# SCUT-BIP-Lab/SplatCo

Hardware: AMD Instinct MI355X
Metric: rasterizer fwd+bwd Msplats/s @1080p; PSNR-match vs ref (higher is better)
Workload: dtype f32; 1 GPU; cfg1: 1M synthetic Gaussians (seed 0), 1 view 1920x1080 per GPU, GaussianRasterizer forward+backward, colors_precomp + scale/rotation path; gaussians=1000000, image=1920x1080, visible=1000000, parallelism=1 view per GPU (mv sharding)

## Files before the change

### splatco_amd/csrc/blend.hip

```cpp
#include <type_traits>

#include "common.h"

namespace scr {

typedef float v2f __attribute__((ext_vector_type(2)));

#ifdef SCR_BLEND_COUNT
__device__ __forceinline__ void count_sub_blocks(unsigned long long m, unsigned long long (&len)[4]) {
    len[0] += (m & 0x000000000f0f0f0full) != 0ull;
    len[1] += (m & 0x00000000f0f0f0f0ull) != 0ull;
    len[2] += (m & 0x0f0f0f0f00000000ull) != 0ull;
    len[3] += (m & 0xf0f0f0f000000000ull) != 0ull;
}
#define SCR_COUNT_SUB(m) (count_sub_blocks((m), sub_), count_sub_blocks((m), subc_))
#define SCR_COUNT_CHUNK_END(i)                                                                             \
    do {                                                                                                   \
        const unsigned long long a_ = subc_[0] > subc_[1] ? subc_[0] : subc_[1], b_ = subc_[2] > subc_[3] ? subc_[2] : subc_[3]; \
        cnt_[(i)] += a_ > b_ ? a_ : b_;                                                                    \
        subc_[0] = subc_[1] = subc_[2] = subc_[3] = 0;                                                     \
    } while (0)
#define SCR_COUNT_SUB_FLUSH(i_sum, i_max)                                                                  \
    do {                                                                                                   \
        cnt_[(i_sum)] += sub_[0] + sub_[1] + sub_[2] + sub_[3];                                            \
        const unsigned long long a_ = sub_[0] > sub_[1] ? sub_[0] : sub_[1], b_ = sub_[2] > sub_[3] ? sub_[2] : sub_[3]; \
        cnt_[(i_max)] += a_ > b_ ? a_ : b_;                                                                \
    } while (0)
#endif
#ifdef SCR_BLEND_COUNT
__device__ unsigned long long g_blend_counters[16];
#define SCR_COUNT(i, v) (cnt_[(i)] += (unsigned long long)(v))
#define SCR_COUNT_DECL unsigned long long cnt_[16] = {}, sub_[4] = {}, subc_[4] = {}
#define SCR_COUNT_FLUSH(lane)                                                        \
    if ((lane) == 0)                                                                 \
        for (int q_ = 0; q_ < 16; ++q_)                                              \
            if (cnt_[q_]) atomicAdd(&g_blend_counters[q_], cnt_[q_])
#else
#define SCR_COUNT(i, v) ((void)0)
#define SCR_COUNT_SUB(m) ((void)0)
#define SCR_COUNT_CHUNK_END(i) ((void)0)
#define SCR_COUNT_SUB_FLUSH(a, b) ((void)0)
#define SCR_COUNT_DECL ((void)0)
#define SCR_COUNT_FLUSH(lane) ((void)0)
#endif

__device__ __forceinline__ float fast_exp(float x) {
    const float p = x * 1.4426950408889634f;
    const float g = __builtin_amdgcn_exp2f(p);
    const float r = __builtin_fmaf(-p, 0.6931471805599453f, x);
    return __builtin_fmaf(g, r, g);
}

__device__ __forceinline__ uint32_t lanes_below(unsigned long long ballot) {
    return __builtin_amdgcn_mbcnt_hi((uint32_t)(ballot >> 32), __builtin_amdgcn_mbcnt_lo((uint32_t)ballot, 0u));
}

__global__ void __launch_bounds__(1024)
tile_order_kernel(int tiles, int gx, const uint32_t* __restrict__ ranges, uint32_t* __restrict__ order,
                  unsigned long long* __restrict__ ordered, unsigned long long* __restrict__ first) {
    __shared__ uint32_t hist[1024], start[1024], wsum[16];
    __shared__ uint32_t s_max, cnt[NUM_XCD];
    const int me = blockIdx.x;
    hist[threadIdx.x] = 0;
    if (threadIdx.x == 0) s_max = 1;
    if (threadIdx.x < NUM_XCD) cnt[threadIdx.x] = 0;
    __syncthreads();
    uint32_t mx = 0, mine[NUM_XCD] = {};
    for (int t = threadIdx.x; t < tiles; t += 1024) {
        const int x = xcd_of_tile(t, gx);
#pragma unroll
        for (int q = 0; q < NUM_XCD; ++q) mine[q] += x == q;
        if (x == me) mx = max(mx, ranges[2 * t + 1] - ranges[2 * t]);
    }
#pragma unroll
    for (int q = 0; q < NUM_XCD; ++q)
        if (mine[q]) atomicAdd(&cnt[q], mine[q]);
    if (mx) atomicMax(&s_max, mx);
    __syncthreads();
    uint32_t off = 0;
    for (int q = 0; q < me; ++q) off += cnt[q];
    const float scale = 1023.0f / (float)s_max;
    for (int t = threadIdx.x; t < tiles; t += 1024) {
        if (xcd_of_tile(t, gx) != me) continue;
        const uint32_t n = ranges[2 * t + 1] - ranges[2 * t];
        atomicAdd(&hist[1023 - min(1023u, (uint32_t)((float)n * scale))], 1u);
    }
    __syncthreads();
    {
        const int lane = threadIdx.x & 63, w = threadIdx.x >> 6;
        uint32_t v = hist[threadIdx.x], inc = v;
#pragma unroll
        for (int d = 1; d < 64; d <<= 1) {
            const uint32_t o = __shfl_up(inc, d, 64);
            if (lane >= d) inc += o;
        }
        if (lane == 63) wsum[w] = inc;
        __syncthreads();
        uint32_t base = 0;
        for (int q = 0; q < w; ++q) base += wsum[q];
        start[threadIdx.x] = base + inc - v;
    }
    __syncthreads();
    for (int t = threadIdx.x; t < tiles; t += 1024) {
        if (xcd_of_tile(t, gx) != me) continue;
        const uint32_t n = ranges[2 * t + 1] - ranges[2 * t];
        order[off + atomicAdd(&start[1023 - min(1023u, (uint32_t)((float)n * scale))], 1u)] = (uint32_t)t;
    }
    if (threadIdx.x == 0) {
        first[me] = off;
        if (me == NUM_XCD - 1) first[NUM_XCD] = off + cnt[me];
        if (me == 0) *ordered = 1;
    }
}

__device__ __forceinline__ int blend_tile(int slot, int tiles, const uint32_t* __restrict__ order,
                                          const unsigned long long* __restrict__ total) {
    const int xcd = slot % NUM_XCD, j = slot / NUM_XCD;
    if (total[2]) {
        const uint32_t f = (uint32_t)total[4 + xcd], e = (uint32_t)total[5 + xcd];
        return f + j < e ? (int)order[f + j] : -1;
    }
    const int chunk = (tiles + NUM_XCD - 1) / NUM_XCD;
    const int t = xcd * chunk + j;
    return j < chunk && t < tiles ? t : -1;
}

template <bool AUX>
__device__ __forceinline__ void masked_blend(unsigned long long live, float w, float cr, float cg, float cb, float z, float Tn,
                                             uint32_t j, float& C0, float& C1, float& C2, float& D, float& T, uint32_t& last) {
    if constexpr (AUX)
        asm volatile("s_mov_b64 exec, %6\n\t"
                     "v_fmac_f32_e32 %0, %7, %11\n\t"
                     "v_fmac_f32_e32 %1, %8, %11\n\t"
                     "v_fmac_f32_e32 %2, %9, %11\n\t"
                     "v_fmac_f32_e32 %3, %10, %11\n\t"
                     "v_mov_b32_e32 %4, %12\n\t"
                     "v_mov_b32_e32 %5, %13\n\t"
                     "s_mov_b64 exec, -1"
                     : "+v"(C0), "+v"(C1), "+v"(C2), "+v"(D), "+v"(T), "+v"(last)
                     : "s"(live), "v"(cr), "v"(cg), "v"(cb), "v"(z), "v"(w), "v"(Tn), "v"(j));
    else
        asm volatile("s_mov_b64 exec, %5\n\t"
                     "v_fmac_f32_e32 %0, %6, %9\n\t"
                     "v_fmac_f32_e32 %1, %7, %9\n\t"
                     "v_fmac_f32_e32 %2, %8, %9\n\t"
                     "v_mov_b32_e32 %3, %10\n\t"
                     "v_mov_b32_e32 %4, %11\n\t"
                     "s_mov_b64 exec, -1"
                     : "+v"(C0), "+v"(C1), "+v"(C2), "+v"(T), "+v"(last)
                     : "s"(live), "v"(cr), "v"(cg), "v"(cb), "v"(w), "v"(Tn), "v"(j));
}

constexpr int FCHUNK = 64;

template <bool SAFE, bool AUX>
__global__ void __launch_bounds__(64)
blend_forward_kernel(int W, int H, int gx, int tiles, const uint32_t* __restrict__ order, const unsigned long long* __restrict__ total,
                     const uint32_t* __restrict__ ranges,
                     const uint32_t* __restrict__ point_list, const uint8_t* __restrict__ qmask,
                     const float4* __restrict__ rec, const float* __restrict__ bg,
                     float* __restrict__ out_color, float* __restrict__ final_T,
                     uint32_t* __restrict__ n_contrib, float* __restrict__ out_depth, float* __restrict__ out_alpha) {
    constexpr int NF = AUX ? 6 : 5;
    __shared__ float4 sp[NF][FCHUNK / 2];
    const int quad = (blockIdx.x / NUM_XCD) & 3;
    const int t = blend_tile((int)(blockIdx.x % NUM_XCD + (blockIdx.x / (4 * NUM_XCD)) * NUM_XCD), tiles, order, total);
    if (t < 0) return;
    const int lane = threadIdx.x;
    const int px = (t % gx) * TILE + (quad & 1) * 8 + (lane & 7);
    const int py = (t / gx) * TILE + (quad >> 1) * 8 + (lane >> 3);
    const bool inside = px < W && py < H;
    const float pxf = (float)px, pyf = (float)py;
    const uint32_t lo = ranges[2 * t], n = ranges[2 * t + 1] - lo;
    unsigned long long done = lanes(!inside);
    SCR_COUNT_DECL;
    float T = 1.0f, C0 = 0.0f, C1 = 0.0f, C2 = 0.0f;
    float D = 0.0f;
    float c099 = 0.99f;
    asm volatile("" : "+v"(c099));
    uint32_t last = 0;

    uint32_t m_next = 0, id_next = 0;
    bool sel_cur = false;
    float4 r0 = make_float4(0, 0, 0, 0), r1 = r0;
    float r2x = 0.0f, r2y = 0.0f;
    auto load_mask_id = [&](uint32_t base, uint32_t& m, uint32_t& id) {
        uint32_t i = base + lane;
        bool have = i < n;
        m = have ? ((qmask[lo + i] >> quad) & 1u) : 0u;
        id = have ? point_list[lo + i] : 0u;
    };
    auto gather = [&](uint32_t m, uint32_t id) {
        sel_cur = m != 0;
        if (sel_cur) {
            r0 = rec[3 * (size_t)id];
            r1 = rec[3 * (size_t)id + 1];
            r2x = rec[3 * (size_t)id + 2].x;
            if (AUX) r2y = rec[3 * (size_t)id + 2].y;
        }
    };
    for (int i = lane; i < NF * (FCHUNK / 2); i += WAVE) (&sp[0][0])[i] = make_float4(0, 0, 0, 0);
    uint32_t m0, id0;
    load_mask_id(0, m0, id0);
    gather(m0, id0);
    load_mask_id(FCHUNK, m_next, id_next);

    for (uint32_t base = 0; base < n; base += FCHUNK) {
        const unsigned long long bal = __builtin_amdgcn_ballot_w64(sel_cur);
        const int cnt = __builtin_popcountll(bal);
        if (sel_cur) {
            const uint32_t pos = lanes_below(bal), q = pos >> 1, h = pos & 1;
            float* f0 = (float*)&sp[0][q];
            float* f1 = (float*)&sp[1][q];
            float* f2 = (float*)&sp[2][q];
            float* f3 = (float*)&sp[3][q];
            float* f4 = (float*)&sp[4][q];
            f0[h] = r0.x; f0[2 + h] = r0.y;
            f1[h] = r0.z; f1[2 + h] = r0.w;
            f2[h] = r1.x; f2[2 + h] = r1.y;
            f3[h] = r1.z; f3[2 + h] = r1.w;
            f4[h] = r2x;  f4[2 + h] = __uint_as_float(base + lane + 1);
            if (AUX) ((float*)&sp[NF - 1][q])[h] = r2y;
        }
        gather(m_next, id_next);
        load_mask_id(base + 2 * FCHUNK, m_next, id_next);
        __syncthreads();
        auto group = [&](const int k, auto npairs) {
            constexpr int NP = decltype(npairs)::value, NS = 2 * NP;
            v2f power[NP], al[NP];
            float4 p3[NP], p4[NP];
            float2 p5[NP];
#pragma unroll
            for (int h = 0; h < NP; ++h) {
                const int q = (k >> 1) + h;
                const float4 p0 = sp[0][q], p1 = sp[1][q], p2 = sp[2][q];
                p3[h] = sp[3][q];
                p4[h] = sp[4][q];
                if (AUX) p5[h] = *(const float2*)&sp[NF - 1][q];
                const v2f dx = v2f{p0.x, p0.y} - pxf, dy = v2f{p0.z, p0.w} - pyf;
                const v2f A = {p1.x, p1.y}, B = {p1.z, p1.w}, Cq = {p2.x, p2.y}, o = {p2.z, p2.w};
                power[h] = __builtin_elementwise_fma(dx, __builtin_elementwise_fma(A, dx, B * dy), (Cq * dy) * dy);
                al[h] = o * v2f{fast_exp(power[h].x), fast_exp(power[h].y)};
            }
            float alpha[NS], pw[NS], om[NS];
#pragma unroll
            for (int h = 0; h < NP; ++h) {
                alpha[2 * h] = vmin(c099, al[h].x); alpha[2 * h + 1] = vmin(c099, al[h].y);
                pw[2 * h] = power[h].x; pw[2 * h + 1] = power[h].y;
            }
#pragma unroll
            for (int u = 0; u < NS; ++u) om[u] = 1.0f - alpha[u];
            unsigned long long hit[NS], anyh = 0ull;
#pragma unroll
            for (int u = 0; u < NS; ++u) {
                hit[u] = (k + u < cnt) ? (lanes(!(pw[u] > 0.0f)) & lanes(!(alpha[u] < 1.0f / 255.0f))) : 0ull;
                anyh |= hit[u];
            }
#ifdef SCR_BLEND_COUNT
            for (int u = 0; u < NS; ++u)
                if (k + u < cnt) {
                    SCR_COUNT(0, 1);
                    SCR_COUNT(2, __builtin_popcountll(done & lanes(inside)));
                    SCR_COUNT(3, (anyh & ~done) == 0ull);
                }
#endif
            if ((anyh & ~done) == 0ull) return;
#pragma unroll
            for (int u = 0; u < NS; ++u) {
                const int h = u >> 1;
                const float cr = (u & 1) ? p3[h].y : p3[h].x, cg = (u & 1) ? p3[h].w : p3[h].z;
                const float cb = (u & 1) ? p4[h].y : p4[h].x, cj = (u & 1) ? p4[h].w : p4[h].z;
                const unsigned long long hm = hit[u] & ~done;
                const float Tn = T * om[u];
                const unsigned long long stop = lanes(Tn < 0.0001f) & hm;
                done |= stop;
                const unsigned long long live = hm & ~stop;
                SCR_COUNT(1, __builtin_popcountll(live));
                SCR_COUNT_SUB(live);
                const float w = alpha[u] * T;
                masked_blend<AUX>(live, w, cr, cg, cb, AUX ? ((u & 1) ? p5[h].y : p5[h].x) : 0.0f, Tn, __float_as_uint(cj),
                                  C0, C1, C2, D, T, last);
            }
        };
        int k = 0;
        for (; k + 2 < cnt; k += 4) group(k, std::integral_constant<int, 2>{});
        if (k < cnt) group(k, std::integral_constant<int, 1>{});
        SCR_COUNT_CHUNK_END(6);
        if (~done == 0ull) break;
        __syncthreads();
    }
    SCR_COUNT_SUB_FLUSH(4, 5);
    SCR_COUNT_FLUSH(lane);
    if (inside) {
        size_t pix = (size_t)py * W + px, hw = (size_t)H * W;
        out_color[pix] = __builtin_fmaf(T, bg[0], C0);
        out_color[hw + pix] = __builtin_fmaf(T, bg[1], C1);
        out_color[2 * hw + pix] = __builtin_fmaf(T, bg[2], C2);
        final_T[pix] = T;
        n_contrib[pix] = last;
        if (AUX) {
            out_depth[pix] = D;
            out_alpha[pix] = 1.0f - T;
        }
    }
}

#define SCR_DPP(d, s, ctrl) "v_add_f32_dpp " d ", " s ", " s " " ctrl "\n\t"
__device__ __forceinline__ void column_fold(float& s0, float& s1, float& s2, float t0, float t1, float t2) {
    asm volatile("s_nop 1\n\t"
                 SCR_DPP("%0", "%0", "row_shl:4 row_mask:0xf bank_mask:0x5")
                 SCR_DPP("%1", "%1", "row_shl:4 row_mask:0xf bank_mask:0x5")
                 SCR_DPP("%2", "%2", "row_shl:4 row_mask:0xf bank_mask:0x5")
                 SCR_DPP("%0", "%3", "row_shr:4 row_mask:0xf bank_mask:0xa")
                 SCR_DPP("%1", "%4", "row_shr:4 row_mask:0xf bank_mask:0xa")
                 SCR_DPP("%2", "%5", "row_shr:4 row_mask:0xf bank_mask:0xa")
                 SCR_DPP("%0", "%0", "quad_perm:[2,3,0,1] row_mask:0xf bank_mask:0xf")
                 SCR_DPP("%1", "%1", "quad_perm:[2,3,0,1] row_mask:0xf bank_mask:0xf")
                 SCR_DPP("%2", "%2", "quad_perm:[2,3,0,1] row_mask:0xf bank_mask:0xf")
                 SCR_DPP("%0", "%0", "quad_perm:[1,0,3,2] row_mask:0xf bank_mask:0xf")
                 SCR_DPP("%1", "%1", "quad_perm:[1,0,3,2] row_mask:0xf bank_mask:0xf")
                 SCR_DPP("%2", "%2", "quad_perm:[1,0,3,2] row_mask:0xf bank_mask:0xf")
                 "s_nop 1"
                 : "+v"(s0), "+v"(s1), "+v"(s2)
                 : "v"(t0), "v"(t1), "v"(t2));
}
constexpr int TCS = WAVE + 4;

struct PixState {
    float T, dLp0, dLp1, dLp2;
    float behind, last_alpha, d_last;
    float dLd, dLa;
};
template <bool SAFE, bool AUX>
__device__ __forceinline__ void splat_pixel_grad(PixState& s, float T, float4 b, float cb, float z, float G, float alpha,
                                                 unsigned long long hit, float& Y, float& w) {
#pragma clang fp contract(fast)
    w = alpha * T;
    s.behind = SAFE ? s.last_alpha * s.d_last + (1.0f - s.last_alpha) * s.behind : s.last_alpha * (s.d_last - s.behind) + s.behind;
    float d = b.z * s.dLp0 + b.w * s.dLp1 + cb * s.dLp2;
    if (AUX) d += z * s.dLd + s.dLa;
    if (SAFE) d = sel(hit, d, 0.0f);
    Y = G * (T * (d - s.behind));
    if (SAFE) Y = sel(hit, Y, 0.0f);
    s.last_alpha = alpha;
    s.d_last = d;
}
__device__ __forceinline__ void group_transmittance(float& T, const float (&om)[4], float (&Tu)[4]) {
#pragma clang fp contract(off)
    const float P = ((om[0] * om[1]) * om[2]) * om[3];
    float r = __builtin_amdgcn_rcpf(P);
    r = __builtin_fmaf(__builtin_fmaf(-P, r, 1.0f), r, r);
    const float q = T * r;
    Tu[3] = __builtin_fmaf(__builtin_fmaf(-q, P, T), r, q);
    Tu[2] = Tu[3] * om[3];
    Tu[1] = Tu[2] * om[2];
    Tu[0] = Tu[1] * om[1];
    T = Tu[3];
}

typedef float f4_t __attribute__((ext_vector_type(4)));
__device__ __forceinline__ void store16_dword_aligned(void* p, float4 v) {
    const f4_t q = {v.x, v.y, v.z, v.w};
    asm volatile("global_store_dwordx4 %0, %1, off" : : "v"(p), "v"(q) : "memory");
}

template <bool AUX> struct RecTail { float x; };
template <> struct RecTail<true> { float x, z; };
constexpr int BCH = 64;
constexpr int BWD_MIN_WAVES = 4;
constexpr int ACC_BUFS = 2;

constexpr int BWD_MIN_WAVES_AUX = 3;
template <bool SAFE, bool AUX>
__global__ void __launch_bounds__(256, AUX ? BWD_MIN_WAVES_AUX : BWD_MIN_WAVES)
blend_backward_kernel(int W, int H, int gx, int tiles, const uint32_t* __restrict__ order, const unsigned long long* __restrict__ total,
                      const uint32_t* __restrict__ ranges,
                      const uint32_t* __restrict__ point_list, const uint32_t* __restrict__ gm_index,
                      const uint2* __restrict__ gm_base,
                      const uint8_t* __restrict__ qmask, const float4* __restrict__ rec,
                      const float* __restrict__ bg, const float* __restrict__ final_T,
                      const uint32_t* __restrict__ n_contrib, const float* __restrict__ dL_dpix,
                      GradRec* __restrict__ grad_rec, unsigned long long* __restrict__ cut_key, unsigned long long stamp,
                      uint8_t* __restrict__ has_rec, const float* __restrict__ dL_ddepth, const float* __restrict__ dL_dalpha,
                      float* __restrict__ grad_z) {
    __shared__ float4 st[4][3][BCH + 4];
    __shared__ float4 accA[ACC_BUFS][4][BCH], accB[ACC_BUFS][4][BCH];
    __shared__ float accC[ACC_BUFS][4][BCH];
    __shared__ float accD[ACC_BUFS][4][BCH];
    __shared__ __attribute__((aligned(16))) float tr[4][8 * TCS];
    __shared__ uint32_t wave_max[4];
    const int t = blend_tile((int)blockIdx.x, tiles, order, total);
    if (t < 0) return;
    const uint32_t lo = ranges[2 * t], n = ranges[2 * t + 1] - lo;
    if (n == 0) return;
    const int wave = threadIdx.x >> 6, lane = threadIdx.x & 63;
    const int qx0 = (t % gx) * TILE + (wave & 1) * 8, qy0 = (t / gx) * TILE + (wave >> 1) * 8;
    const int px = qx0 + (lane >> 3), py = qy0 + (lane & 7);
    const bool inside = px < W && py < H;
    const float pxf = (float)px, pyf = (float)py;
    const float qx0f = (float)qx0, qy0f = (float)qy0;
    const size_t pix = (size_t)py * W + px, hw = (size_t)H * W;
    const uint32_t last = inside ? n_contrib[pix] : 0u;
    PixState ps;
    ps.T = inside ? final_T[pix] : 0.0f;
    ps.dLp0 = ps.dLp1 = ps.dLp2 = 0.0f;
    if (inside) {
        ps.dLp0 = dL_dpix[pix];
        ps.dLp1 = dL_dpix[hw + pix];
        ps.dLp2 = dL_dpix[2 * hw + pix];
    }
    ps.behind = (bg[0] * ps.dLp0 + bg[1] * ps.dLp1) + bg[2] * ps.dLp2;
    ps.last_alpha = ps.d_last = 0.0f;
    if (AUX) {
        ps.dLd = inside && dL_ddepth ? dL_ddepth[pix] : 0.0f;
        ps.dLa = inside && dL_dalpha ? dL_dalpha[pix] : 0.0f;
    }
    float c099 = 0.99f;
    asm volatile("" : "+v"(c099));
    SCR_COUNT_DECL;
    const int rcol = lane >> 3, rx = lane & 7;
    constexpr int WZ = AUX ? 3 : 0;
    float wgt[AUX ? 4 : 3][8];
#pragma unroll
    for (int y = 0; y < 8; ++y) {
        wgt[0][y] = 1.0f; wgt[1][y] = (float)y; wgt[2][y] = (float)(y * y);
        if (AUX) wgt[WZ][y] = 0.0f;
        if (rcol >= 4) {
            const bool in = qx0 + rx < W && qy0 + y < H;
            const size_t q = (size_t)(qy0 + y) * W + (size_t)(qx0 + rx);
#pragma unroll
            for (int c = 0; c < 3; ++c) wgt[c][y] = in ? dL_dpix[c * hw + q] : 0.0f;
            if (AUX) wgt[WZ][y] = in && dL_ddepth ? dL_ddepth[q] : 0.0f;
        }
    }
    const float xw = rcol < 4 ? (float)rx : 0.0f;
    float* const trw = &tr[wave][0];
    const float* const trr = trw + rcol * TCS + 8 * rx;
    const int rkind = rcol >= 4 ? 2 : (lane >> 2) & 1;
    const bool rstore = (lane & 3) == 0 && (rcol < 4 || ((lane >> 2) & 1) == 0);
    const bool rstore_z = AUX && (lane & 3) == 0 && rcol >= 4 && ((lane >> 2) & 1) == 1;
    const int rcu = rcol & 3;
    const unsigned long long rcu1 = lanes(rcu == 1), rcu2 = lanes(rcu == 2), rcu3 = lanes(rcu == 3);
    char* const accA0 = (char*)&accA[0][wave][0];
    char* const accB0 = (char*)&accB[0][wave][0];
    char* const rdst0 = rkind == 0 ? accA0 : rkind == 1 ? accA0 + 4 : accB0 + 8;
    char* const rdst1 = rkind == 0 ? accA0 + 8 : rkind == 1 ? accA0 + 12 : accB0 + 12;
    char* const rdst2 = rkind == 0 ? accB0 + 4 : rkind == 1 ? accB0 : (char*)&accC[0][wave][0];
    const uint32_t rstride2 = rkind == 2 ? 4u : 16u;
    constexpr uint32_t PAR_A = sizeof(float4) * 4 * BCH, PAR_C = sizeof(float) * 4 * BCH;
    const uint32_t rpar2 = rkind == 2 ? PAR_C : PAR_A;
    uint32_t wm = last;
#pragma unroll
    for (int d = 32; d > 0; d >>= 1) wm = max(wm, (uint32_t)__shfl_xor((int)wm, d, WAVE));
    if (lane == 0) wave_max[wave] = wm;
    if (lane < 9) st[wave][lane / 3][lane % 3] = make_float4(0, 0, 0, 0);
    __syncthreads();
    const uint32_t wmax0 = wave_max[0], wmax1 = wave_max[1], wmax2 = wave_max[2], wmax3 = wave_max[3];
    const uint32_t max_last = max(max(wmax0, wmax1), max(wmax2, wmax3));
    const uint32_t wave_last = wave == 0 ? wmax0 : wave == 1 ? wmax1 : wave == 2 ? wmax2 : wmax3;
    const int nround = (int)((n + BCH - 1) / BCH);
    const int live_top = max_last ? (int)((max_last - 1) / BCH) : -1;

    constexpr int CUT_MIN_ROUNDS = 3;
    const bool cut = nround - 1 - live_top >= CUT_MIN_ROUNDS;
    if (threadIdx.x == 0) {
        unsigned long long ck = ~0ull;
        if (cut) {
            const uint32_t idc = point_list[lo + (uint32_t)(live_top + 1) * BCH];
            ck = ((unsigned long long)__float_as_uint(rec[3 * (size_t)idc + 2].y) << 32) | idc;
            cut_key[tiles] = stamp;
        }
        cut_key[t] = ck;
    }
    const uint32_t tile_x = (uint32_t)(t % gx), tile_y = (uint32_t)(t / gx);
    auto gm_of = [&](uint32_t pos, uint32_t id) -> uint32_t {
        if (gm_index) return gm_index[pos];
        const uint2 b = gm_base[id];
        return b.x + tile_y * b.y + tile_x;
    };
    if (!cut && (AUX || wave < 3))
        for (int ci = nround - 1; ci > live_top; --ci) {
            const uint32_t i = (uint32_t)ci * BCH + lane;
            if (i < n && qmask[lo + i] != 0) {
                const uint32_t gmi = gm_of(lo + i, point_list[lo + i]);
                GradRec& gr = grad_rec[gmi];
                if (wave == 0) store16_dword_aligned(&gr.a, make_float4(0, 0, 0, 0));
                else if (wave == 1) store16_dword_aligned(&gr.b, make_float4(0, 0, 0, 0));
                else if (!AUX || wave == 2) gr.c = 0.0f;
                else grad_z[gmi] = 0.0f;
            }
        }

    uint32_t m_next = 0, id_next = 0, slot_next = 0;
    uint32_t m_cur = 0, slot_cur = 0, id_cur = 0;
    bool sel_cur = false;
    float4 r0 = make_float4(0, 0, 0, 0), r1 = r0;
    RecTail<AUX> r2 = {};
    auto load_meta = [&](int ci, uint32_t& m, uint32_t& id, uint32_t& slot) {
        const uint32_t i = (uint32_t)ci * BCH + lane;
        const bool have = ci >= 0 && i < n;
        m = have ? qmask[lo + i] : 0u;
        id = have ? point_list[lo + i] : 0u;
        slot = have ? gm_of(lo + i, id) : 0u;
    };
    auto gather = [&](int ci, uint32_t m, uint32_t id, uint32_t slot) {
        const uint32_t i = (uint32_t)ci * BCH + lane;
        sel_cur = ((m >> wave) & 1u) && i < wave_last;
        m_cur = m;
        slot_cur = slot;
        id_cur = id;
        if (sel_cur) {
            r0 = rec[3 * (size_t)id];
            r1 = rec[3 * (size_t)id + 1];
            r2.x = rec[3 * (size_t)id + 2].x;
            if constexpr (AUX) r2.z = rec[3 * (size_t)id + 2].y;
        }
    };
    if (live_top >= 0) {
        uint32_t m0, id0, sl0;
        load_meta(live_top, m0, id0, sl0);
        gather(live_top, m0, id0, sl0);
        load_meta(live_top - 1, m_next, id_next, slot_next);
    }
    for (int ci = live_top; ci >= 0; --ci) {
        const uint32_t base = (uint32_t)ci * BCH;
        const int last_rel = (int)last - (int)base;
        const unsigned long long bal = __builtin_amdgcn_ballot_w64(sel_cur);
        const int cnt = __builtin_popcountll(bal);
        if (sel_cur) {
            const uint32_t pos = lanes_below(bal);
            st[wave][0][pos + 3] = r0;
            st[wave][1][pos + 3] = r1;
            float r2z = 0.0f;
            if constexpr (AUX) r2z = r2.z;
            st[wave][2][pos + 3] = make_float4(r2.x, __uint_as_float((uint32_t)lane), r2z, 0.0f);
        }
        const uint32_t m_this = m_cur, slot_this = slot_cur, id_this = id_cur;
        gather(ci - 1, m_next, id_next, slot_next);
        load_meta(ci - 2, m_next, id_next, slot_next);
        const int par = ci & 1;
        auto group = [&](const int k, auto tail) {
            constexpr bool TAIL = decltype(tail)::value;
            float Y[4], Wt[4];
            uint32_t jj[4] = {0u, 0u, 0u, 0u};
            unsigned long long hits[4] = {0ull, 0ull, 0ull, 0ull};
            float4 ra[4], rb[4];
            float2 rc[4];
            float rz[4] = {0.0f, 0.0f, 0.0f, 0.0f};
#pragma unroll
            for (int u = 0; u < 4; ++u) {
                ra[u] = st[wave][0][k + 3 - u];
                rb[u] = st[wave][1][k + 3 - u];
                rc[u] = *(const float2*)&st[wave][2][k + 3 - u];
                if (AUX) rz[u] = st[wave][2][k + 3 - u].z;
            }
            float Gs[4], al[4], om[4], Tu[4];
#pragma unroll
            for (int u = 0; u < 4; ++u) {
                if (TAIL && k - u < 0) {
                    Gs[u] = al[u] = 0.0f;
                    om[u] = 1.0f;
                    SCR_COUNT(13, 1);
                    continue;
                }
                const float4 a = ra[u], b = rb[u];
                const uint32_t j = __float_as_uint(rc[u].y);
                const float dx = a.x - pxf, dy = a.y - pyf;
                const float power = __builtin_fmaf(dx, __builtin_fmaf(a.z, dx, a.w * dy), (b.x * dy) * dy);
                const float ar = b.y * fast_exp(power);
                const unsigned long long hit = lanes((int)j < last_rel) & lanes(!(power > 0.0f)) & lanes(!(ar < 1.0f / 255.0f));
                SCR_COUNT(8, 1);
                SCR_COUNT(9, __builtin_popcountll(hit));
                SCR_COUNT_SUB(hit);
                SCR_COUNT(10, __builtin_popcountll(lanes(!((int)j < last_rel)) & lanes(inside)));
                SCR_COUNT(11, __builtin_popcountll(lanes(!(power > 0.0f)) & lanes(!(ar < 1.0f / 255.0f)) & lanes(inside)));
                Gs[u] = sel(hit, ar, 0.0f);
                al[u] = vmin(c099, Gs[u]);
                om[u] = 1.0f - al[u];
                if (SAFE) hits[u] = hit;
                jj[u] = j;
            }
            group_transmittance(ps.T, om, Tu);
#pragma unroll
            for (int u = 0; u < 4; ++u) {
                if (TAIL && k - u < 0) {
                    Y[u] = Wt[u] = 0.0f;
                    continue;
                }
                splat_pixel_grad<SAFE, AUX>(ps, Tu[u], rb[u], rc[u].x, rz[u], Gs[u], al[u], hits[u], Y[u], Wt[u]);
            }
            float s0, s1, s2;
            {
                asm volatile("" ::: "memory");
#pragma unroll
                for (int u = 0; u < 4; ++u) {
                    trw[u * TCS + lane] = Y[u];
                    trw[(4 + u) * TCS + lane] = Wt[u];
                }
                asm volatile("" ::: "memory");
                const float4 va = *(const float4*)trr, vb = *(const float4*)(trr + 4);
                asm volatile("" ::: "memory");
                const float v[8] = {va.x, va.y, va.z, va.w, vb.x, vb.y, vb.z, vb.w};
                float e0 = wgt[0][0] * v[0], e1 = wgt[1][0] * v[0], e2 = wgt[2][0] * v[0];
                float o0 = wgt[0][1] * v[1], o1 = wgt[1][1] * v[1], o2 = wgt[2][1] * v[1];
#pragma unroll
                for (int y = 2; y < 8; y += 2) {
                    e0 = __builtin_fmaf(wgt[0][y], v[y], e0);
                    e1 = __builtin_fmaf(wgt[1][y], v[y], e1);
                    e2 = __builtin_fmaf(wgt[2][y], v[y], e2);
                    o0 = __builtin_fmaf(wgt[0][y + 1], v[y + 1], o0);
                    o1 = __builtin_fmaf(wgt[1][y + 1], v[y + 1], o1);
                    o2 = __builtin_fmaf(wgt[2][y + 1], v[y + 1], o2);
                }
                s0 = e0 + o0; s1 = e1 + o1; s2 = e2 + o2;
                float t0 = xw * s0;
                if (AUX) {
                    float e3 = wgt[WZ][0] * v[0], o3 = wgt[WZ][1] * v[1];
#pragma unroll
                    for (int y = 2; y < 8; y += 2) {
                        e3 = __builtin_fmaf(wgt[WZ][y], v[y], e3);
                        o3 = __builtin_fmaf(wgt[WZ][y + 1], v[y + 1], o3);
                    }
                    t0 = __builtin_fmaf(xw, s0, e3 + o3);
                }
                const float t1 = xw * t0, t2 = xw * s1;
                column_fold(s0, s1, s2, t0, t1, t2);
            }
            if (rstore && (!TAIL || k - rcu >= 0)) {
                const uint32_t jw = sel(rcu3, jj[3], sel(rcu2, jj[2], sel(rcu1, jj[1], jj[0])));
                *(float*)(rdst0 + par * PAR_A + jw * 16u) = s0;
                *(float*)(rdst1 + par * PAR_A + jw * 16u) = s1;
                *(float*)(rdst2 + par * rpar2 + jw * rstride2) = s2;
            }
            if (AUX && rstore_z && (!TAIL || k - rcu >= 0)) {
                const uint32_t jw = sel(rcu3, jj[3], sel(rcu2, jj[2], sel(rcu1, jj[1], jj[0])));
                accD[par][wave][jw] = s0;
            }
        };
        int k = cnt - 1;
        for (; k >= 3; k -= 4) group(k, std::false_type{});
        if (k >= 0) group(k, std::true_type{});
        SCR_COUNT_CHUNK_END(7);
        asm volatile("s_waitcnt lgkmcnt(0)" ::: "memory");
        if (lane < cnt) {
            const float4 ra = st[wave][0][lane + 3];
            const uint32_t j = __float_as_uint(st[wave][2][lane + 3].y);
            const float a = ra.x - qx0f, b = ra.y - qy0f;
            const float4 A = accA[par][wave][j], B = accB[par][wave][j];
            const float M0 = A.x, Mx = A.y, My = A.z, Mxx = A.w, Mxy = B.x, Myy = B.y;
            const float t1 = a * M0 - Mx, t2 = b * M0 - My;
            accA[par][wave][j] = make_float4(t1, t2, a * (t1 - Mx) + Mxx, (a * t2 - b * Mx) + Mxy);
            accB[par][wave][j] = make_float4(b * (t2 - My) + Myy, M0, B.z, B.w);
        }
        __syncthreads();
        if (wave < 3 && base + lane < n && m_this != 0) {
            const uint32_t i = base + lane;
            float4 r = make_float4(0, 0, 0, 0);
            auto part = [&](int w) {
                return wave == 0 ? accA[par][w][lane] : wave == 1 ? accB[par][w][lane]
                                                                  : make_float4(accC[par][w][lane], 0.0f, 0.0f, 0.0f);
            };
            if (((m_this >> 0) & 1u) && i < wmax0) { const float4 x = part(0); r.x += x.x; r.y += x.y; r.z += x.z; r.w += x.w; }
            if (((m_this >> 1) & 1u) && i < wmax1) { const float4 x = part(1); r.x += x.x; r.y += x.y; r.z += x.z; r.w += x.w; }
            if (((m_this >> 2) & 1u) && i < wmax2) { const float4 x = part(2); r.x += x.x; r.y += x.y; r.z += x.z; r.w += x.w; }
            if (((m_this >> 3) & 1u) && i < wmax3) { const float4 x = part(3); r.x += x.x; r.y += x.y; r.z += x.z; r.w += x.w; }
            GradRec& gr = grad_rec[slot_this];
            if (wave == 0) store16_dword_aligned(&gr.a, r);
            else if (wave == 1) store16_dword_aligned(&gr.b, r);
            else {
                gr.c = r.x;
                if (has_rec) has_rec[id_this] = 1;
            }
        }
        if (AUX && wave == 3 && base + lane < n && m_this != 0) {
            const uint32_t i = base + lane;
            float r = 0.0f;
            if (((m_this >> 0) & 1u) && i < wmax0) r += accD[par][0][lane];
            if (((m_this >> 1) & 1u) && i < wmax1) r += accD[par][1][lane];
            if (((m_this >> 2) & 1u) && i < wmax2) r += accD[par][2][lane];
            if (((m_this >> 3) & 1u) && i < wmax3) r += accD[par][3][lane];
            grad_z[slot_this] = r;
        }
    }
    SCR_COUNT_SUB_FLUSH(14, 15);
    SCR_COUNT_FLUSH(lane);
}

static int blend_slots_per_xcd(const Grid& g) {
    int cnt[NUM_XCD] = {};
    for (int t = 0; t < g.tiles; ++t) ++cnt[xcd_of_tile(t, g.gx)];
    int m = (g.tiles + NUM_XCD - 1) / NUM_XCD;
    for (int q = 0; q < NUM_XCD; ++q) m = cnt[q] > m ? cnt[q] : m;
    return m;
}

void launch_blend_forward(const KSettings& ks, const GeomView& gv, const BinView& bv, const ImgView& iv,
                          float* out_color, float* out_depth, float* out_alpha, bool longest_first, bool safe,
                          hipStream_t st) {
    Grid g(ks.H, ks.W);
    if (longest_first)
        tile_order_kernel<<<NUM_XCD, 1024, 0, st>>>(g.tiles, g.gx, gv.ranges, gv.tile_count, gv.total + 2, gv.total + 4);
    const bool aux = out_depth != nullptr;
    auto kernel = aux ? (safe ? blend_forward_kernel<true, true> : blend_forward_kernel<false, true>)
                      : (safe ? blend_forward_kernel<true, false> : blend_forward_kernel<false, false>);
    kernel<<<(unsigned)blend_slots_per_xcd(g) * NUM_XCD * 4, 64, 0, st>>>(
        ks.W, ks.H, g.gx, g.tiles, gv.tile_count, gv.total, gv.ranges, bv.point_list, bv.qmask, gv.rec, ks.bg, out_color, iv.final_T,
        iv.n_contrib, out_depth, out_alpha);
}

void launch_blend_backward(const KSettings& ks, const GeomView& gv, const BinView& bv, const ImgView& iv,
                           const float* dL_dcolor, const float* dL_ddepth, const float* dL_dalpha, GradRec* grad_rec,
                           float* grad_z, unsigned long long stamp, bool deep, bool flags, bool safe, hipStream_t st) {
    Grid g(ks.H, ks.W);
    const bool gm_from_base = deep;
    if (flags) { ZeroList z; z.add(gv.has_rec, ((size_t)gv.P + 3) / 4 * 4, st); launch_zero(z, st); }
    const bool aux = grad_z != nullptr;
    auto kernel = aux ? (safe ? blend_backward_kernel<true, true> : blend_backward_kernel<false, true>)
                      : (safe ? blend_backward_kernel<true, false> : blend_backward_kernel<false, false>);
    kernel<<<(unsigned)blend_slots_per_xcd(g) * NUM_XCD, 256, 0, st>>>(
        ks.W, ks.H, g.gx, g.tiles, gv.tile_count, gv.total, gv.ranges, bv.point_list, gm_from_base ? nullptr : bv.gm_index, gv.gm_base,
        bv.qmask, gv.rec, ks.bg,
        iv.final_T, iv.n_contrib, dL_dcolor, grad_rec, iv.cut_key, stamp, flags ? gv.has_rec : nullptr, dL_ddepth, dL_dalpha,
        grad_z);
}

}

#ifdef SCR_BLEND_COUNT
extern "C" int scr_tool_blend_counters(unsigned long long* out16, int reset) {
    if (out16 && hipMemcpyFromSymbol(out16, HIP_SYMBOL(scr::g_blend_counters), 16 * 8) != hipSuccess) return 1;
    if (reset) {
        unsigned long long z[16] = {};
        if (hipMemcpyToSymbol(HIP_SYMBOL(scr::g_blend_counters), z, 16 * 8) != hipSuccess) return 1;
    }
    return 0;
}
#endif
```

Before: 1095 Msplats/s.

## Read per-lane Gaussian slot from LDS, batch masked combine, split transpose layout

Adds three compile-time options to the backward blend kernel, all enabled by default (SCR_BWD_ITEMS=14). Each lane reads its slot index directly from the staged LDS record instead of a chain of selects. The four per-wave partial accumulators are combined with a single exec-masked inline-asm add sequence instead of branchy conditional adds. The transpose scratch buffer uses a split column layout to change LDS bank mapping. It also extends the debug counter set. The inline asm with exec manipulation risks correctness and register pressure, and the new layout could change bank conflicts either way.

```diff
diff --git a/splatco_amd/csrc/blend.hip b/splatco_amd/csrc/blend.hip
--- a/splatco_amd/csrc/blend.hip
+++ b/splatco_amd/csrc/blend.hip
@@ -28,12 +28,13 @@
     } while (0)
 #endif
 #ifdef SCR_BLEND_COUNT
-__device__ unsigned long long g_blend_counters[16];
+constexpr int SCR_NCOUNT = 20;
+__device__ unsigned long long g_blend_counters[SCR_NCOUNT];
 #define SCR_COUNT(i, v) (cnt_[(i)] += (unsigned long long)(v))
-#define SCR_COUNT_DECL unsigned long long cnt_[16] = {}, sub_[4] = {}, subc_[4] = {}
+#define SCR_COUNT_DECL unsigned long long cnt_[SCR_NCOUNT] = {}, sub_[4] = {}, subc_[4] = {}
 #define SCR_COUNT_FLUSH(lane)                                                        \
     if ((lane) == 0)                                                                 \
-        for (int q_ = 0; q_ < 16; ++q_)                                              \
+        for (int q_ = 0; q_ < SCR_NCOUNT; ++q_)                                              \
             if (cnt_[q_]) atomicAdd(&g_blend_counters[q_], cnt_[q_])
 #else
 #define SCR_COUNT(i, v) ((void)0)
@@ -324,7 +325,15 @@
                  : "+v"(s0), "+v"(s1), "+v"(s2)
                  : "v"(t0), "v"(t1), "v"(t2));
 }
+#ifndef SCR_BWD_ITEMS
+#define SCR_BWD_ITEMS 14
+#endif
+constexpr bool BWD_LANE_POS = (SCR_BWD_ITEMS & 2) != 0, BWD_BATCH_COMBINE = (SCR_BWD_ITEMS & 4) != 0,
+               BWD_TR_SPLIT = (SCR_BWD_ITEMS & 8) != 0;
+
 constexpr int TCS = WAVE + 4;
+constexpr int TR_WORDS = BWD_TR_SPLIT ? 8 * WAVE + 4 : 8 * TCS;
+__device__ __forceinline__ constexpr int tr_col(int c) { return BWD_TR_SPLIT ? WAVE * (c >> 1) + (c & 1) * (4 * WAVE + 4) : c * TCS; }
 
 struct PixState {
     float T, dLp0, dLp1, dLp2;
@@ -364,6 +373,51 @@
     asm volatile("global_store_dwordx4 %0, %1, off" : : "v"(p), "v"(q) : "memory");
 }
 
+__device__ __forceinline__ void masked_add4(float4& r, const float4 (&x)[4], const unsigned long long (&c)[4]) {
+    unsigned long long keep;
+    asm volatile("s_mov_b64 %4, exec\n\t"
+                 "s_mov_b64 exec, %5\n\t"
+                 "v_add_f32_e32 %0, %0, %9\n\t"
+                 "v_add_f32_e32 %1, %1, %10\n\t"
+                 "v_add_f32_e32 %2, %2, %11\n\t"
+                 "v_add_f32_e32 %3, %3, %12\n\t"
+                 "s_mov_b64 exec, %6\n\t"
+                 "v_add_f32_e32 %0, %0, %13\n\t"
+                 "v_add_f32_e32 %1, %1, %14\n\t"
+                 "v_add_f32_e32 %2, %2, %15\n\t"
+                 "v_add_f32_e32 %3, %3, %16\n\t"
+                 "s_mov_b64 exec, %7\n\t"
+                 "v_add_f32_e32 %0, %0, %17\n\t"
+                 "v_add_f32_e32 %1, %1, %18\n\t"
+                 "v_add_f32_e32 %2, %2, %19\n\t"
+                 "v_add_f32_e32 %3, %3, %20\n\t"
+                 "s_mov_b64 exec, %8\n\t"
+                 "v_add_f32_e32 %0, %0, %21\n\t"
+                 "v_add_f32_e32 %1, %1, %22\n\t"
+                 "v_add_f32_e32 %2, %2, %23\n\t"
+                 "v_add_f32_e32 %3, %3, %24\n\t"
+                 "s_mov_b64 exec, %4"
+                 : "+v"(r.x), "+v"(r.y), "+v"(r.z), "+v"(r.w), "=&s"(keep)
+                 : "s"(c[0]), "s"(c[1]), "s"(c[2]), "s"(c[3]),
+                   "v"(x[0].x), "v"(x[0].y), "v"(x[0].z), "v"(x[0].w), "v"(x[1].x), "v"(x[1].y), "v"(x[1].z), "v"(x[1].w),
+                   "v"(x[2].x), "v"(x[2].y), "v"(x[2].z), "v"(x[2].w), "v"(x[3].x), "v"(x[3].y), "v"(x[3].z), "v"(x[3].w));
+}
+__device__ __forceinline__ void masked_add4(float& r, const float (&x)[4], const unsigned long long (&c)[4]) {
+    unsigned long long keep;
+    asm volatile("s_mov_b64 %1, exec\n\t"
+                 "s_mov_b64 exec, %2\n\t"
+                 "v_add_f32_e32 %0, %0, %6\n\t"
+                 "s_mov_b64 exec, %3\n\t"
+                 "v_add_f32_e32 %0, %0, %7\n\t"
+                 "s_mov_b64 exec, %4\n\t"
+                 "v_add_f32_e32 %0, %0, %8\n\t"
+                 "s_mov_b64 exec, %5\n\t"
+                 "v_add_f32_e32 %0, %0, %9\n\t"
+                 "s_mov_b64 exec, %1"
+                 : "+v"(r), "=&s"(keep)
+                 : "s"(c[0]), "s"(c[1]), "s"(c[2]), "s"(c[3]), "v"(x[0]), "v"(x[1]), "v"(x[2]), "v"(x[3]));
+}
+
 template <bool AUX> struct RecTail { float x; };
 template <> struct RecTail<true> { float x, z; };
 constexpr int BCH = 64;
@@ -387,7 +441,7 @@
     __shared__ float4 accA[ACC_BUFS][4][BCH], accB[ACC_BUFS][4][BCH];
     __shared__ float accC[ACC_BUFS][4][BCH];
     __shared__ float accD[ACC_BUFS][4][BCH];
-    __shared__ __attribute__((aligned(16))) float tr[4][8 * TCS];
+    __shared__ __attribute__((aligned(16))) float tr[4][TR_WORDS];
     __shared__ uint32_t wave_max[4];
     const int t = blend_tile((int)blockIdx.x, tiles, order, total);
     if (t < 0) return;
@@ -435,11 +489,12 @@
     }
     const float xw = rcol < 4 ? (float)rx : 0.0f;
     float* const trw = &tr[wave][0];
-    const float* const trr = trw + rcol * TCS + 8 * rx;
+    const float* const trr = trw + tr_col(rcol) + 8 * rx;
     const int rkind = rcol >= 4 ? 2 : (lane >> 2) & 1;
     const bool rstore = (lane & 3) == 0 && (rcol < 4 || ((lane >> 2) & 1) == 0);
     const bool rstore_z = AUX && (lane & 3) == 0 && rcol >= 4 && ((lane >> 2) & 1) == 1;
     const int rcu = rcol & 3;
+    const float4* const rpos = &st[wave][2][3 - rcu];
     const unsigned long long rcu1 = lanes(rcu == 1), rcu2 = lanes(rcu == 2), rcu3 = lanes(rcu == 3);
     char* const accA0 = (char*)&accA[0][wave][0];
     char* const accB0 = (char*)&accB[0][wave][0];
@@ -554,6 +609,8 @@
                 rc[u] = *(const float2*)&st[wave][2][k + 3 - u];
                 if (AUX) rz[u] = st[wave][2][k + 3 - u].z;
             }
+            uint32_t jpos = 0u;
+            if (BWD_LANE_POS) jpos = __float_as_uint(rpos[k].y);
             float Gs[4], al[4], om[4], Tu[4];
 #pragma unroll
             for (int u = 0; u < 4; ++u) {
@@ -594,8 +651,8 @@
                 asm volatile("" ::: "memory");
 #pragma unroll
                 for (int u = 0; u < 4; ++u) {
-                    trw[u * TCS + lane] = Y[u];
-                    trw[(4 + u) * TCS + lane] = Wt[u];
+                    trw[tr_col(u) + lane] = Y[u];
+                    trw[tr_col(4 + u) + lane] = Wt[u];
                 }
                 asm volatile("" ::: "memory");
                 const float4 va = *(const float4*)trr, vb = *(const float4*)(trr + 4);
@@ -627,19 +684,27 @@
                 column_fold(s0, s1, s2, t0, t1, t2);
             }
             if (rstore && (!TAIL || k - rcu >= 0)) {
-                const uint32_t jw = sel(rcu3, jj[3], sel(rcu2, jj[2], sel(rcu1, jj[1], jj[0])));
+                const uint32_t jw = BWD_LANE_POS ? jpos : sel(rcu3, jj[3], sel(rcu2, jj[2], sel(rcu1, jj[1], jj[0])));
                 *(float*)(rdst0 + par * PAR_A + jw * 16u) = s0;
                 *(float*)(rdst1 + par * PAR_A + jw * 16u) = s1;
                 *(float*)(rdst2 + par * rpar2 + jw * rstride2) = s2;
             }
             if (AUX && rstore_z && (!TAIL || k - rcu >= 0)) {
-                const uint32_t jw = sel(rcu3, jj[3], sel(rcu2, jj[2], sel(rcu1, jj[1], jj[0])));
+                const uint32_t jw = BWD_LANE_POS ? jpos : sel(rcu3, jj[3], sel(rcu2, jj[2], sel(rcu1, jj[1], jj[0])));
                 accD[par][wave][jw] = s0;
             }
         };
         int k = cnt - 1;
         for (; k >= 3; k -= 4) group(k, std::false_type{});
         if (k >= 0) group(k, std::true_type{});
+#ifdef SCR_BLEND_COUNT
+        {
+            const bool no_edge = ~(lanes(last_rel >= BCH) | lanes(last_rel <= 0)) == 0ull;
+            SCR_COUNT(16, cnt != 0);
+            SCR_COUNT(17, cnt != 0 && no_edge);
+            SCR_COUNT(18, no_edge ? cnt : 0);
+        }
+#endif
         SCR_COUNT_CHUNK_END(7);
         asm volatile("s_waitcnt lgkmcnt(0)" ::: "memory");
         if (lane < cnt) {
@@ -660,10 +725,23 @@
                 return wave == 0 ? accA[par][w][lane] : wave == 1 ? accB[par][w][lane]
                                                                   : make_float4(accC[par][w][lane], 0.0f, 0.0f, 0.0f);
             };
+            if constexpr (BWD_BATCH_COMBINE) {
+                const unsigned long long took[4] = {lanes(((m_this >> 0) & 1u) && i < wmax0), lanes(((m_this >> 1) & 1u) && i < wmax1),
+                                                    lanes(((m_this >> 2) & 1u) && i < wmax2), lanes(((m_this >> 3) & 1u) && i < wmax3)};
+                if (wave == 2) {
+                    const float x[4] = {accC[par][0][lane], accC[par][1][lane], accC[par][2][lane], accC[par][3][lane]};
+                    masked_add4(r.x, x, took);
+                } else {
+                    const float4* const p = wave == 0 ? &accA[par][0][lane] : &accB[par][0][lane];
+                    const float4 x[4] = {p[0], p[BCH], p[2 * BCH], p[3 * BCH]};
+                    masked_add4(r, x, took);
+                }
+            } else {
             if (((m_this >> 0) & 1u) && i < wmax0) { const float4 x = part(0); r.x += x.x; r.y += x.y; r.z += x.z; r.w += x.w; }
             if (((m_this >> 1) & 1u) && i < wmax1) { const float4 x = part(1); r.x += x.x; r.y += x.y; r.z += x.z; r.w += x.w; }
             if (((m_this >> 2) & 1u) && i < wmax2) { const float4 x = part(2); r.x += x.x; r.y += x.y; r.z += x.z; r.w += x.w; }
             if (((m_this >> 3) & 1u) && i < wmax3) { const float4 x = part(3); r.x += x.x; r.y += x.y; r.z += x.z; r.w += x.w; }
+            }
             GradRec& gr = grad_rec[slot_this];
             if (wave == 0) store16_dword_aligned(&gr.a, r);
             else if (wave == 1) store16_dword_aligned(&gr.b, r);
@@ -675,10 +753,17 @@
         if (AUX && wave == 3 && base + lane < n && m_this != 0) {
             const uint32_t i = base + lane;
             float r = 0.0f;
+            if constexpr (BWD_BATCH_COMBINE) {
+                const unsigned long long took[4] = {lanes(((m_this >> 0) & 1u) && i < wmax0), lanes(((m_this >> 1) & 1u) && i < wmax1),
+                                                    lanes(((m_this >> 2) & 1u) && i < wmax2), lanes(((m_this >> 3) & 1u) && i < wmax3)};
+                const float x[4] = {accD[par][0][lane], accD[par][1][lane], accD[par][2][lane], accD[par][3][lane]};
+                masked_add4(r, x, took);
+            } else {
             if (((m_this >> 0) & 1u) && i < wmax0) r += accD[par][0][lane];
             if (((m_this >> 1) & 1u) && i < wmax1) r += accD[par][1][lane];
             if (((m_this >> 2) & 1u) && i < wmax2) r += accD[par][2][lane];
             if (((m_this >> 3) & 1u) && i < wmax3) r += accD[par][3][lane];
+            }
             grad_z[slot_this] = r;
         }
     }
@@ -727,11 +812,11 @@
 }
 
 #ifdef SCR_BLEND_COUNT
-extern "C" int scr_tool_blend_counters(unsigned long long* out16, int reset) {
-    if (out16 && hipMemcpyFromSymbol(out16, HIP_SYMBOL(scr::g_blend_counters), 16 * 8) != hipSuccess) return 1;
+extern "C" int scr_tool_blend_counters(unsigned long long* out20, int reset) {
+    if (out20 && hipMemcpyFromSymbol(out20, HIP_SYMBOL(scr::g_blend_counters), scr::SCR_NCOUNT * 8) != hipSuccess) return 1;
     if (reset) {
-        unsigned long long z[16] = {};
-        if (hipMemcpyToSymbol(HIP_SYMBOL(scr::g_blend_counters), z, 16 * 8) != hipSuccess) return 1;
+        unsigned long long z[scr::SCR_NCOUNT] = {};
+        if (hipMemcpyToSymbol(HIP_SYMBOL(scr::g_blend_counters), z, scr::SCR_NCOUNT * 8) != hipSuccess) return 1;
     }
     return 0;
 }
```

Result: faster. 1119 Msplats/s (median of 6 runs) (+2.2%).
